# mikel-zhobro/pytorch3d_pointops

Measured on AMD Instinct MI355X. Metric: Mpoint-pairs/s (+ %HBM roofline) knn_points B=32 N=65536 K=16 @1/2/4/8 GPU, higher is better.
Workload: dtype f32; 1 GPU; knn_points B=32 N=M=65536 K=16 D=3 fp32 per GPU (BASELINE.json configs[1]); splitmix64 uniform [0,1)^3 clouds, p1 != p2, full lengths, norm=2; clouds_per_gpu=32, clouds_total=32

## Files before the change

### pytorch3d_pointops_amd/csrc/grid.h

```cpp
#pragma once
#include <float.h>
#include <math.h>

#include "knn_grid.h"

namespace pointops {

constexpr int kGMax = 1024;
constexpr int kEdgeStride = kGMax + 2;
constexpr int kGridWave = 64;
constexpr int kNumXcd = 8;
constexpr int kCoarseMax = 1024;
constexpr int kCrowdedMax = 64;
constexpr int kFineLogMax = 12;
constexpr int kOrderG = 16, kOrderBins = kOrderG * kOrderG * kOrderG;
constexpr int kSortedPad = 32;

inline int lane_search_workgroups(int64_t N, int P1) {
  const int64_t chunks = (N * ceil_div(P1, kGridWave) + 7) / 8 * 8;
  return (int)(chunks < 2048 ? 2048 : (chunks > (1 << 20) ? (1 << 20) : chunks));
}

struct GridCloud {
  float lo[3];
// ... 2 lines not shown
  int ncell;
  int len1, len2;
  int use_grid;
  int same;
  int mshift, nmicro;
};

struct RefinedCell {
  int start, count;
  int s;
  int pool_off;
  float lo[3], scale[3];
};

struct GridWs {
  GridCloud* cloud;
  int* chunk_prefix;
  float* edges;
  int* cell_start;
  int* coarse_count;
  int* bin_of;
  int* bin_first;
  int* nbins;
  int* coarse_cursor;
  int* coarse_start;
  float4* sorted;
  int* coarse_ticket;
  int* crowded_count;
  int* crowded_list;
  int* fine_count;
  int* prank;
  int* qrank;
  float4* qtmp;
  float4* qsorted;
  int* order_table;
  int* fb_count;
  int* fb_list;
  unsigned* fb_kth;
  int* fb2_count;
  int* fb2_list;
  int* fb3_count;
  int* fb3_list;
  unsigned* bbox;
  float* bbox_part;
  int* grid_flag;
  int* refine_ref;
  RefinedCell* rdesc;
  int* rcount;
  int* pool;
  int* pool_top;
  float4* sorted_tmp;
  int* box_count;
  int* box_list;
  int rdesc_cap, pool_cap;
  float c_target;
  int cell_cap;
  int ball;
};

struct GridBuild {
  float c_target;
  float h_min;
  float ball_radius;
  int ball_K;
  float ball_factor;
  bool same;
  int refine;
};

constexpr int kRefineMaxS = 32;

__host__ __device__ inline int refine_threshold(float c_target) {
  const float r = 28.0f * c_target;
  return r < 64.0f ? 64 : (int)r;
}
constexpr int kDeferFactor = 4;

__device__ __forceinline__ int sub_of(float x, float lo, float scale, int s) {
  const float t = (x - lo) * scale;
  int c = (t < (float)s) ? (int)t : s - 1;
  if (!(t >= 0.0f)) c = 0;
  return c;
}

size_t grid_carve(GridWs* ws, char* base, int64_t N, int64_t P1, int64_t P2, float c_target, bool ball = false);
int grid_build(const KnnArgs& a, const GridWs& ws, const GridBuild& b);
int grid_build_queries(const KnnArgs& a, const GridWs& ws, bool same, int level);
int grid_refine(const KnnArgs& a, const GridWs& ws);

__device__ __forceinline__ int cell_of(float x, float lo, float inv_h, int G) {
  const float t = (x - lo) * inv_h;
  int c = (t < (float)G) ? (int)t : G - 1;
  if (!(t >= 0.0f)) c = 0;
  return c;
}
__device__ __forceinline__ unsigned fkey(float f) {
  const unsigned u = __float_as_uint(f);
  return (u & 0x80000000u) ? ~u : (u | 0x80000000u);
}
__device__ __forceinline__ float funkey(unsigned k) {
  return __uint_as_float((k & 0x80000000u) ? (k & 0x7fffffffu) : ~k);
}
__device__ __forceinline__ float prev_float(float x) { return funkey(fkey(x) - 1u); }

template <int D>
__device__ __forceinline__ void load_point3(const float* __restrict__ p, float& x, float& y, float& z) {
  x = p[0];
  y = D > 1 ? p[1] : 0.0f;
  z = D > 2 ? p[2] : 0.0f;
}

__device__ __forceinline__ void point_cells(const GridCloud& g, float x, float y, float z, int& cx, int& cy,
                                            int& cz) {
  cx = cell_of(x, g.lo[0], g.inv_h, g.G[0]);
  cy = cell_of(y, g.lo[1], g.inv_h, g.G[1]);
  cz = cell_of(z, g.lo[2], g.inv_h, g.G[2]);
}
__device__ __forceinline__ int cell_index(const GridCloud& g, int cx, int cy, int cz) {
  return (cz * g.G[1] + cy) * g.G[0] + cx;
}
__device__ __forceinline__ int cell_id(const GridCloud& g, float x, float y, float z) {
  int cx, cy, cz;
  point_cells(g, x, y, z, cx, cy, cz);
  return cell_index(g, cx, cy, cz);
}

__device__ __forceinline__ int clamp_len(int64_t len, int P) {
  const int l = (int)len;
  return l < 0 ? 0 : (l > P ? P : l);
}

template <int BLOCK, typename Fn>
__device__ __forceinline__ void for_each4(const float4* __restrict__ src, int count, Fn fn) {
  for (int i0 = 0; i0 < count; i0 += 4 * BLOCK) {
    float4 p[4];
#pragma unroll
    for (int u = 0; u < 4; ++u) {
      const int j = i0 + u * BLOCK + (int)threadIdx.x;
      p[u] = j < count ? src[j] : make_float4(0.0f, 0.0f, 0.0f, 0.0f);
    }
#pragma unroll
    for (int u = 0; u < 4; ++u) {
      const int j = i0 + u * BLOCK + (int)threadIdx.x;
      fn(p[u], j, j < count);
    }
  }
}

template <int NORM>
__device__ __forceinline__ float face_bound(float t) {
  return NORM == 1 ? t : t * t;
}

template <int D, int NORM>
__device__ __forceinline__ float point_dist(float qx, float qy, float qz, const float4 c) {
  float d;
  if (NORM == 1) {
    d = __builtin_fabsf(qx - c.x);
    if (D > 1) d = d + __builtin_fabsf(qy - c.y);
    if (D > 2) d = d + __builtin_fabsf(qz - c.z);
  } else {
    const float dx = qx - c.x;
    d = dx * dx;
    if (D > 1) {
      const float dy = qy - c.y;
      d = d + dy * dy;
    }
    if (D > 2) {
      const float dz = qz - c.z;
      d = d + dz * dz;
    }
  }
  return d;
}

template <int NORM>
__device__ __forceinline__ float box_lower_bound(const GridCloud& g, const float* __restrict__ ed, float qx, float qy,
// ... 53 lines not shown
```

### pytorch3d_pointops_amd/csrc/grid_build.hip

```cpp
#include <stdlib.h>

#include "grid.h"
#include "wave.h"

namespace pointops {

constexpr int kSetupBlock = 1024;
constexpr int kCoarsePoints = 1024;

__device__ __forceinline__ int64_t coarse_row(int n, int set) { return ((int64_t)n * 2 + set) * (kCoarseMax + 1); }

__device__ __forceinline__ void reset_set_state(const GridWs& ws, int n, int set) {
  const int tid = threadIdx.x;
  if (tid == 0) {
    ws.coarse_ticket[n * 2 + set] = 0;
    ws.crowded_count[n * 2 + set] = 0;
    ws.nbins[n * 2 + set] = 0;
  }
  for (int t = tid; t < kCoarseMax + 1; t += kSetupBlock) {
    ws.coarse_count[coarse_row(n, set) + t] = 0;
    ws.coarse_cursor[coarse_row(n, set) + t] = 0;
  }
}
__device__ __forceinline__ void reset_query_state(const GridWs& ws, int n) {
// ... 175 lines not shown
    if (ok && any_active && !one_cell) {
      for (int d = 0; d < 3; ++d)
        if (active[d]) h = fmaxf(h, e[d] * (1.0f / ((float)kGMax - 0.5f)));
      for (int it = 0; it < 64; ++it) {
        inv_h = 1.0f / h;
        if (!(inv_h > 0.0f && inv_h <= FLT_MAX)) {
          ok = false;
          break;
        }
        long long cells = 1;
        for (int d = 0; d < 3; ++d) {
          G[d] = 1;
          if (active[d]) {
            const float t = e[d] * inv_h;
            G[d] = (t < (float)kGMax) ? (int)t + 1 : kGMax;
            if (G[d] < 1) G[d] = 1;
          }
          cells *= G[d];
        }
        if (cells <= (long long)ws.cell_cap && cells <= ((long long)kCoarseMax << kFineLogMax)) break;
        h *= 1.2599211f;
      }
      if ((long long)G[0] * G[1] * G[2] > (long long)ws.cell_cap ||
          (long long)G[0] * G[1] * G[2] > ((long long)kCoarseMax << kFineLogMax))
        ok = false;
    }
    for (int d = 0; d < 3; ++d) {
      g.lo[d] = lo[d];
      g.G[d] = G[d];
      s_hi[d] = hi[d];
    }
    g.inv_h = inv_h;
    g.ncell = G[0] * G[1] * G[2];
    g.len1 = len1;
    g.len2 = len2;
    g.mshift = 0;
    while (((g.ncell - 1) >> g.mshift) + 1 > kCoarseMax) ++g.mshift;
    g.nmicro = ((g.ncell - 1) >> g.mshift) + 1;
    if (g.mshift > kFineLogMax) ok = false;
    g.use_grid = ok ? 1 : 0;
    g.same = same;
    s_g = g;
    ws.cloud[n] = g;
    const float qnan = __uint_as_float(0x7fc00000u);
    ws.sorted[(int64_t)n * (P2 + kSortedPad) + P2] = make_float4(qnan, qnan, qnan, 0.0f);
    ws.grid_flag[n] = g.use_grid;
    ws.rcount[n] = 0;
    ws.pool_top[n] = 0;
  }
  reset_set_state(ws, n, 0);
  reset_query_state(ws, n);
  __syncthreads();
  if (s_g.use_grid) {
    float* __restrict__ ed = ws.edges + (int64_t)n * 3 * kEdgeStride;
    for (int t = tid; t < 3 * kEdgeStride; t += kSetupBlock) {
      const int d = t / kEdgeStride, c = t - d * kEdgeStride;
      const int G = s_g.G[d];
      ed[t] = (c <= G) ? edge_bisect(c, s_g.lo[d], s_hi[d], s_g.inv_h, G) : __builtin_inff();
    }
  }
}


__device__ void grid_chunk_prefix(const GridWs& ws, int N) {
  const int lane = threadIdx.x & (kWave - 1);
  int acc = 0;
  if (lane == 0) ws.chunk_prefix[0] = 0;
  for (int n0 = 0; n0 < N; n0 += kWave) {
    const int n = n0 + lane;
    int items = 0;
    if (n < N) {
      const GridCloud g = ws.cloud[n];
      if (g.use_grid) items = (g.len1 + kGridWave - 1) / kGridWave;
    }
    const int inc = wave_inclusive_sum(items);
    if (n < N) ws.chunk_prefix[n + 1] = acc + inc;
    acc += __shfl(inc, kWave - 1, kWave);
  }
}

constexpr int kPartBlock = 1024;
constexpr int kCountPerThread = 16;
constexpr int kScatterPerThread = 4;
constexpr int kSortBlock = 256;
constexpr int kHashBits = 12, kHashSlots = 1 << kHashBits, kHashProbes = 8;
constexpr int kCrowded = 8192;
constexpr int kCrowdedSlice = 4096;
constexpr int kFineMax = 1 << kFineLogMax;
static_assert(kCoarseMax == kPartBlock, "the count launch's last tile scans one micro-bin per thread");

__device__ __forceinline__ void unsearched_row(const GridWs& ws, const GridCloud& g, int n, int i, int P, int K,
                                               int64_t* __restrict__ idxs, float* __restrict__ dists) {
  if (i < P && i >= g.len1) {
    int64_t* __restrict__ zi = idxs + ((int64_t)n * P + i) * K;
    float* __restrict__ zd = dists + ((int64_t)n * P + i) * K;
    const int64_t pad = ws.ball ? -1 : 0;
    for (int k = 0; k < K; ++k) {
      zi[k] = pad;
      zd[k] = 0.0f;
    }
  } else if (i < g.len1 && !g.use_grid && !ws.ball) {
    const int pos = atomicAdd(ws.fb2_count + n, 1);
    ws.fb2_list[(int64_t)n * P + pos] = i;
  }
}

__device__ __forceinline__ void bin_cells(const GridCloud& g, const int* bfirst, int b, int& f0, int& nf) {
  f0 = bfirst[b] << g.mshift;
  nf = min((bfirst[b + 1] - bfirst[b]) << g.mshift, g.ncell - f0);
}

// ... 361 lines not shown
  }
}

static int grid_cell_cap(int64_t P2, float c_target) {
  const int64_t cells = (int64_t)ceil((double)P2 / (double)c_target);
  return (int)(2 * cells + 64);
}

size_t grid_carve(GridWs* ws, char* base, int64_t N, int64_t P1, int64_t P2, float c, bool ball) {
  const int cap = grid_cell_cap(P2, c);
  Carver cv(base);
  GridWs w;
  w.cell_cap = cap;
  w.cloud = (GridCloud*)cv.take(sizeof(GridCloud) * (size_t)N);
  w.chunk_prefix = (int*)cv.take(sizeof(int) * (size_t)(N + 1));
  w.edges = (float*)cv.take(sizeof(float) * (size_t)N * 3 * kEdgeStride);
  w.cell_start = (int*)cv.take(sizeof(int) * (size_t)N * (cap + 1));
  w.coarse_count = (int*)cv.take(sizeof(int) * (size_t)N * 2 * (kCoarseMax + 1));
  w.coarse_cursor = (int*)cv.take(sizeof(int) * (size_t)N * 2 * (kCoarseMax + 1));
  w.coarse_start = (int*)cv.take(sizeof(int) * (size_t)N * 2 * (kCoarseMax + 1));
  w.bin_of = (int*)cv.take(sizeof(int) * (size_t)N * 2 * (kCoarseMax + 1));
  w.bin_first = (int*)cv.take(sizeof(int) * (size_t)N * 2 * (kCoarseMax + 1));
  w.nbins = (int*)cv.take(sizeof(int) * (size_t)N * 2);
  w.coarse_ticket = (int*)cv.take(sizeof(int) * (size_t)N * 2);
  w.crowded_count = (int*)cv.take(sizeof(int) * (size_t)N * 2);
  w.crowded_list = (int*)cv.take(sizeof(int) * (size_t)N * 2 * kCrowdedMax);
  w.fine_count = (int*)cv.take(sizeof(int) * (size_t)N * 2 * cap);
  w.prank = (int*)cv.take(sizeof(int) * (size_t)N * (size_t)P2);
  w.qrank = (int*)cv.take(sizeof(int) * (size_t)N * (size_t)P1);
  w.order_table = (int*)cv.take(ball ? sizeof(int) * (size_t)N * (size_t)((P1 + 2047) / 2048) * kOrderBins : 0);
  w.sorted = (float4*)cv.take(sizeof(float4) * (size_t)N * (size_t)(P2 + kSortedPad));
  w.qsorted = (float4*)cv.take(sizeof(float4) * (size_t)N * (size_t)P1);
  w.fb_count = (int*)cv.take(sizeof(int) * (size_t)N);
  w.fb_list = (int*)cv.take(sizeof(int) * (size_t)N * (size_t)P1);
  w.fb_kth = (unsigned*)cv.take(sizeof(unsigned) * (size_t)N * (size_t)P1);
  w.fb2_count = (int*)cv.take(sizeof(int) * (size_t)N);
  w.fb2_list = (int*)cv.take(sizeof(int) * (size_t)N * (size_t)P1);
  w.fb3_count = (int*)cv.take(sizeof(int) * (size_t)N);
  w.fb3_list = (int*)cv.take(sizeof(int) * (size_t)N * (size_t)P1);
  w.bbox = (unsigned*)cv.take(sizeof(unsigned) * (size_t)N * 8);
  w.bbox_part = (float*)cv.take(sizeof(float) * (size_t)N * 6 * (size_t)((P2 + 2047) / 2048));
  w.grid_flag = (int*)cv.take(sizeof(int) * (size_t)N);
  w.qtmp = (float4*)cv.take(sizeof(float4) * (size_t)N * (size_t)P1);
  w.rdesc_cap = (int)(P2 / 64 + 1);
  w.pool_cap = (int)(4 * P2 + 64);
  w.refine_ref = (int*)cv.take(sizeof(int) * (size_t)N * cap);
  w.rdesc = (RefinedCell*)cv.take(sizeof(RefinedCell) * (size_t)N * (size_t)w.rdesc_cap);
  w.rcount = (int*)cv.take(sizeof(int) * (size_t)N);
  w.pool = (int*)cv.take(sizeof(int) * (size_t)N * (size_t)w.pool_cap);
  w.pool_top = (int*)cv.take(sizeof(int) * (size_t)N);
  w.sorted_tmp = (float4*)cv.take(sizeof(float4) * (size_t)N * (size_t)P2);
  w.box_count = (int*)cv.take(sizeof(int) * (size_t)N);
  w.box_list = (int*)cv.take(sizeof(int) * (size_t)N * (size_t)P1);
  w.c_target = c;
  w.ball = 0;
  if (ws) *ws = w;
  return cv.off;
}

template <int D>
static void build_d(const KnnArgs& a, const GridWs& ws, int sets_mode, int refine) {
  const bool same = sets_mode == 0;
  const unsigned sets = sets_mode == 2 ? 2u : 1u;
  const int zbase = sets_mode == 1 ? 1 : 0;
  const int64_t pmax = same ? a.P2 : sets_mode == 1 ? a.P1 : (a.P2 > a.P1 ? a.P2 : a.P1);
  auto part = [&](auto scatter, auto queries) {
    hipLaunchKernelGGL((grid_partition_kernel<D, scatter, queries>),
                       dim3((unsigned)ceil_div(pmax, kPartBlock * (scatter ? kScatterPerThread : kCountPerThread)),
                            (unsigned)a.N, sets),
                       dim3(kPartBlock), 0, a.stream, a.p2, a.P2, a.p1, a.P1, a.K, ws, zbase, a.idxs, a.dists);
  };
  if (same) {
    part(std::false_type{}, std::false_type{});
    part(std::true_type{}, std::false_type{});
  } else {
    part(std::false_type{}, std::true_type{});
    part(std::true_type{}, std::true_type{});
  }
  const int64_t bins = pmax / kCoarsePoints + ws.cell_cap / kFineMax + 2;
  int64_t wgs = 8192 / (a.N * (int64_t)sets);
  wgs = wgs < 16 ? 16 : (wgs > kCoarseMax ? kCoarseMax : wgs);
  wgs = wgs > bins ? bins : wgs;
  hipLaunchKernelGGL(grid_sort_kernel, dim3((unsigned)wgs, (unsigned)a.N, sets), dim3(kSortBlock), 0, a.stream, ws,
                     (int)a.P1, (int)a.P2, refine, zbase);
}

__global__ __launch_bounds__(kSetupBlock) void grid_requery_kernel(const int64_t* __restrict__ lengths1, int P1, int same,
                                                                GridWs ws) {
  const int n = blockIdx.x, tid = threadIdx.x;
  if (tid == 0) {
    ws.cloud[n].len1 = clamp_len(lengths1[n], P1);
    ws.cloud[n].same = same;
  }
  reset_query_state(ws, n);
}

__global__ __launch_bounds__(kPartBlock) void grid_pad_prefix_kernel(GridWs ws, int P1, int K, int64_t* __restrict__ idxs,
                                                                  float* __restrict__ dists) {
  const int n = blockIdx.y, tid = threadIdx.x;
  if (blockIdx.x == 0 && blockIdx.y == 0 && tid < kWave) grid_chunk_prefix(ws, (int)gridDim.y);
  const GridCloud g = ws.cloud[n];
  if (g.len1 >= P1 && g.use_grid) return;
  constexpr int kTile = kPartBlock * kCountPerThread;
  for (int r = 0; r < kCountPerThread; ++r)
    unsearched_row(ws, g, n, blockIdx.x * kTile + r * kPartBlock + tid, P1, K, idxs, dists);
}

int grid_build_queries(const KnnArgs& a, const GridWs& ws, bool same, int level) {
  hipLaunchKernelGGL(grid_requery_kernel, dim3((unsigned)a.N), dim3(kSetupBlock), 0, a.stream, a.l1, a.P1, same ? 1 : 0,
                     ws);
  if (same || level >= 2) {
    hipLaunchKernelGGL(grid_pad_prefix_kernel, dim3((unsigned)ceil_div(a.P1, kPartBlock * kCountPerThread), (unsigned)a.N),
                       dim3(kPartBlock), 0, a.stream, ws, a.P1, a.K, a.idxs, a.dists);
  } else {
    with_exact<3>(Ints<1, 2, 3>{}, a.D, [&](auto D) { build_d<D>(a, ws, 1, -1); });
  }
  return check_launch("grid build (queries)");
}

int grid_build(const KnnArgs& a, const GridWs& ws, const GridBuild& b) {
  const int bbox_slots = (int)ceil_div(a.P2, kBboxTile);
  hipLaunchKernelGGL(grid_bbox_kernel, dim3((unsigned)bbox_slots, (unsigned)a.N), dim3(kBboxBlock), 0, a.stream, a.p2,
                     a.l2, a.P2, a.D, ws.bbox_part);
  hipLaunchKernelGGL(grid_setup_kernel, dim3((unsigned)a.N), dim3(kSetupBlock), 0, a.stream, a.p2, a.l1, a.l2, a.P1,
                     a.P2, a.D, b.c_target, b.h_min, b.ball_radius, b.ball_K, b.ball_factor, b.same ? 1 : 0, bbox_slots,
                     ws);
  with_exact<3>(Ints<1, 2, 3>{}, a.D, [&](auto D) { build_d<D>(a, ws, b.same ? 0 : 2, b.refine); });
  return check_launch("grid build");
}

}
```

### pytorch3d_pointops_amd/csrc/grid_refine.hip

```cpp
#include "grid.h"
#include "wave.h"

namespace pointops {

constexpr int kRefineBlock = 1024;
constexpr int kRefineWgs = 8;

template <int D>
__global__ __launch_bounds__(kRefineBlock) void grid_refine_build_kernel(GridWs ws, int P2) {
  extern __shared__ int s_hist[];
  __shared__ double s_red[kRefineBlock / kWave][6];
  __shared__ float s_lo[3], s_scale[3];
  __shared__ int s_wsum[kRefineBlock / kWave];
  const int n = blockIdx.y;
  const int tid = threadIdx.x, lane = tid & (kWave - 1), wave = tid / kWave;
  int nref = ws.rcount[n];
  if (nref > ws.rdesc_cap) nref = ws.rdesc_cap;
  float4* __restrict__ rec = ws.sorted + (int64_t)n * (P2 + kSortedPad);
  float4* __restrict__ tmp = ws.sorted_tmp + (int64_t)n * P2;
  for (int r = blockIdx.x; r < nref; r += gridDim.x) {
    RefinedCell* __restrict__ dp = ws.rdesc + (int64_t)n * ws.rdesc_cap + r;
    const int start = dp->start, count = dp->count, s = dp->s;
    if (count <= 0) continue;
    const int nsub = s * s * s;
    double acc[6] = {0, 0, 0, 0, 0, 0};
    for_each4<kRefineBlock>(rec + start, count, [&](const float4 p, int, bool live) {
      if (!live) return;
      const double v[3] = {p.x, p.y, p.z};
#pragma unroll
      for (int d = 0; d < D; ++d) {
        acc[d] += v[d];
        acc[3 + d] += v[d] * v[d];
      }
    });
#pragma unroll
    for (int k = 0; k < 6; ++k) acc[k] = wave_sum(acc[k]);
    __syncthreads();
    if (lane == 0) {
#pragma unroll
      for (int k = 0; k < 6; ++k) s_red[wave][k] = acc[k];
    }
    __syncthreads();
    if (tid < 3) {
      float lo = 0.0f, scale = 0.0f;
      if (tid < D) {
        double sx = 0, sxx = 0;
        for (int w = 0; w < kRefineBlock / kWave; ++w) {
          sx += s_red[w][tid];
          sxx += s_red[w][3 + tid];
        }
        const double mean = sx / count;
        const double var = sxx / count - mean * mean;
        const double sig = var > 0 ? sqrt(var) : 0.0;
        const double half = 2.2 * sig;
        lo = (float)(mean - half);
        const float width = (float)(2.0 * half);
        scale = (width > 0.0f && width <= FLT_MAX) ? (float)s / width : 0.0f;
        if (!(scale > 0.0f && scale <= FLT_MAX)) scale = 0.0f;
        if (!(fabsf(lo) <= FLT_MAX)) {
          lo = 0.0f;
          scale = 0.0f;
        }
      }
      s_lo[tid] = lo;
      s_scale[tid] = scale;
      dp->lo[tid] = lo;
      dp->scale[tid] = scale;
    }
    for (int b = tid; b < nsub; b += kRefineBlock) s_hist[b] = 0;
    __syncthreads();
    const float lx = s_lo[0], ly = s_lo[1], lz = s_lo[2], kx = s_scale[0], ky = s_scale[1], kz = s_scale[2];
    auto sub_index = [&](const float4 p) {
      const int ix = sub_of(p.x, lx, kx, s);
      const int iy = D > 1 ? sub_of(p.y, ly, ky, s) : 0;
      const int iz = D > 2 ? sub_of(p.z, lz, kz, s) : 0;
      return (iz * s + iy) * s + ix;
    };
    for_each4<kRefineBlock>(rec + start, count, [&](const float4 p, int, bool live) {
      if (live) atomicAdd(&s_hist[sub_index(p)], 1);
    });
    __syncthreads();
    int* __restrict__ table = ws.pool + (int64_t)n * ws.pool_cap + dp->pool_off;
    const int per = (nsub + kRefineBlock - 1) / kRefineBlock;
    const int b0 = tid * per, b1 = min(b0 + per, nsub);
    int sum = 0;
    for (int b = b0; b < b1; ++b) sum += s_hist[b];
    int total;
    int run = block_exclusive_sum<kRefineBlock / kWave>(sum, s_wsum, total);
    for (int b = b0; b < b1; ++b) {
      const int cnt = s_hist[b];
      table[b] = run;
      s_hist[b] = run;
      run += cnt;
    }
    if (tid == kRefineBlock - 1) table[nsub] = count;
    __syncthreads();
    for_each4<kRefineBlock>(rec + start, count, [&](const float4 p, int, bool live) {
      if (live) tmp[start + atomicAdd(&s_hist[sub_index(p)], 1)] = p;
    });
    __threadfence_block();
    __syncthreads();
    for_each4<kRefineBlock>(tmp + start, count, [&](const float4 p, int i, bool live) {
      if (live) rec[start + i] = p;
    });
  }
}

int grid_refine(const KnnArgs& a, const GridWs& ws) {
  const size_t lds = sizeof(int) * (size_t)kRefineMaxS * kRefineMaxS * kRefineMaxS;
  const int64_t per_cloud = 256 / (a.N > 0 ? a.N : 1);
  const dim3 grid((unsigned)(per_cloud < kRefineWgs ? kRefineWgs : (per_cloud > 64 ? 64 : per_cloud)), (unsigned)a.N);
  const int rc = with_exact<3>(Ints<1, 2, 3>{}, a.D, [&](auto D) {
    static bool attr[64] = {false};
    int dev = -1;
    const bool known = hipGetDevice(&dev) == hipSuccess && dev >= 0 && dev < 64;
    if (!known || !attr[dev]) {
      if (hipFuncSetAttribute(reinterpret_cast<const void*>(grid_refine_build_kernel<D>),
                              hipFuncAttributeMaxDynamicSharedMemorySize, (int)lds) != hipSuccess)
        return check_launch("grid refine attribute");
      if (known) attr[dev] = true;
    }
    hipLaunchKernelGGL((grid_refine_build_kernel<D>), grid, dim3(kRefineBlock), lds, a.stream, ws, a.P2);
    return POINTOPS_OK;
  });
  if (rc != POINTOPS_OK) return rc;
  return check_launch("grid refine");
}

}
```

### pytorch3d_pointops_amd/csrc/knn_grid.hip

```cpp
#include "debug.h"
#include "grid.h"
#include "knn_grid_search.h"

namespace pointops {

static int grid_kc(int K) { return with_bucket(kGridKC, K, [](auto KC) { return KC.value; }); }

static float knn_cell_target(int K) {
  const int kc = grid_kc(K);
  float c = (kc >= 8 ? 0.4f : 0.625f) * (float)K;
  c *= (float)debug_knob_f("grid_c_scale", 1.0);
  return c < 1.0f ? 1.0f : c;
}

size_t knn_grid_workspace_bytes(int64_t N, int64_t P1, int64_t P2, int64_t K) {
  return grid_carve(nullptr, nullptr, N < 32768 ? N : 32768, P1, P2, knn_cell_target((int)K));
}

static bool grid_quad_mode(int64_t queries, int kc) {
  const long k = debug_knob("grid_quad", -1);
  return k >= 0 ? k != 0 : queries >= (kc >= 32 ? (1 << 18) : (1 << 20));
}

constexpr int64_t kGridBatchSlice = 32768;

int64_t knn_grid_max_points() { return kGridMaxPointsBig; }

static int knn_grid_run_slice(const KnnArgs& a, int norm, void* workspace, int reuse) {
  GridWs ws;
  const float c = knn_cell_target(a.K);
  grid_carve(&ws, (char*)workspace, a.N, a.P1, a.P2, c);
  GridBuild b{};
  b.c_target = c;
  b.same = a.p1 == a.p2 && a.l1 == a.l2 && a.P1 == a.P2 && debug_knob("grid_same", 1) != 0;
  b.refine = (debug_knob("grid_refine", 1) != 0 && a.K <= 64) ? 1 : 0;
  int rc;
  if (reuse > 0) {
    if ((rc = grid_build_queries(a, ws, b.same, reuse)) != POINTOPS_OK) return rc;
  } else {
    if ((rc = grid_build(a, ws, b)) != POINTOPS_OK) return rc;
    if (b.refine && (rc = grid_refine(a, ws)) != POINTOPS_OK) return rc;
  }
  if (a.K > 64) {
    grid_search_wsort(a, ws, norm);
    rc = check_launch("knn_points_idx(grid, long lists)");
    if (rc != POINTOPS_OK) return rc;
    KnnArgs fa = a;
    fa.qlist = ws.fb2_list;
    fa.qcount = ws.fb2_count;
    if ((rc = launch_knn_wide(fa, norm, 1, nullptr)) != POINTOPS_OK) return rc;
    return check_launch("knn_points_idx(grid fallback)");
  }
  const int kc = grid_kc(a.K);
  const bool quad = kc <= 32 && grid_quad_mode(a.N * (int64_t)a.P1, kc);
  const bool big = a.P2 > kGridMaxPoints || debug_knob("grid_big", 0) != 0;
  with_exact<3>(Ints<1, 2, 3>{}, a.D, [&](auto D) {
    (big ? grid_search<D, kRunBitsBig> : grid_search<D, kRunBitsStd>)(a, ws, norm, kc, quad);
  });
  rc = check_launch("knn_points_idx(grid)");
  if (rc != POINTOPS_OK) return rc;
  KnnArgs fa = a;
  fa.qlist = ws.fb2_list;
  fa.qcount = ws.fb2_count;
  if (a.K <= 32) launch_knn_bruteforce(fa, norm);
  else if ((rc = launch_knn_wide(fa, norm, 1, nullptr)) != POINTOPS_OK) return rc;
  return check_launch("knn_points_idx(grid fallback)");
}

int knn_grid_run(const KnnArgs& a, int norm, void* workspace, int reuse) {
  POINTOPS_REQUIRE(a.P2 <= kGridMaxPointsBig, "knn_points_idx(grid): P2 must be <= 2^24 - 16");
  if (a.N <= kGridBatchSlice) return knn_grid_run_slice(a, norm, workspace, reuse);
  for (int64_t n0 = 0; n0 < a.N; n0 += kGridBatchSlice) {
    KnnArgs s = a;
    const bool same_pts = a.p1 == a.p2, same_len = a.l1 == a.l2;
    s.N = a.N - n0 < kGridBatchSlice ? a.N - n0 : kGridBatchSlice;
    s.p1 = a.p1 + n0 * (int64_t)a.P1 * a.D;
    s.p2 = same_pts ? s.p1 : a.p2 + n0 * (int64_t)a.P2 * a.D;
    s.l1 = a.l1 + n0;
    s.l2 = same_len ? s.l1 : a.l2 + n0;
    s.idxs = a.idxs + n0 * (int64_t)a.P1 * a.K;
    s.dists = a.dists + n0 * (int64_t)a.P1 * a.K;
    const int rc = knn_grid_run_slice(s, norm, workspace, 0);
    if (rc != POINTOPS_OK) return rc;
  }
  return POINTOPS_OK;
}

}

extern "C" int pointops_knn_grid_fallback_counts(const void* workspace, int64_t N, int64_t P1, int64_t P2,
                                                 int64_t K, int32_t* counts, void* stream) {
  using namespace pointops;
  POINTOPS_REQUIRE(workspace != nullptr && counts != nullptr && N > 0 && N <= 32768, "knn_grid_fallback_counts: bad arguments");
  GridWs ws;
  grid_carve(&ws, (char*)workspace, N, P1, P2, knn_cell_target((int)K));
  if (hipMemcpyAsync(counts + N, ws.fb2_count, sizeof(int) * (size_t)N, hipMemcpyDeviceToDevice,
                     (hipStream_t)stream) != hipSuccess)
    return check_launch("knn_grid_fallback_counts");
  if (hipMemcpyAsync(counts, ws.fb_count, sizeof(int) * (size_t)N, hipMemcpyDeviceToDevice,
                     (hipStream_t)stream) != hipSuccess)
    return check_launch("knn_grid_fallback_counts");
  return POINTOPS_OK;
}

namespace pointops {
__global__ void grid_stats_kernel(GridWs ws, int N, int32_t* __restrict__ stats) {
  const int n = blockIdx.x * blockDim.x + threadIdx.x;
  if (n >= N) return;
// ... 30 lines not shown
```

### pytorch3d_pointops_amd/csrc/knn_grid_search.h

```cpp
#pragma once
#include "debug.h"
#include "grid.h"
#include "knn_common.h"
#include "sort_net.h"
#include "wave.h"

#include <type_traits>

namespace pointops {

template <int KC>
__device__ __forceinline__ void write_row_f64(const TopKF64<KC>& top, int K, int len2, int64_t* __restrict__ orow_i,
                                              float* __restrict__ orow_d, bool vec16) {
  write_row<KC>(top, K, len2, orow_i, orow_d, vec16);
}

constexpr int kLaneRows = 9;

template <int KC>
struct LaneCfg {
  static constexpr bool kUseQueue = KC >= 8;
  static constexpr int kQueueCap = 16;
  static constexpr int kQueueLds = KC <= 16 ? 15 : 16;
#ifndef POINTOPS_LANE_GROUP
// ... 70 lines not shown
    for (int u = u0; u < u0 + kSub; ++u) c[u] = record(off, u);
    __builtin_amdgcn_sched_barrier(0);
#pragma unroll
    for (int t = 0; t < kSub; ++t) {
      const bool valid = 16 * STRIDE * (u0 + t) < crem;
      if (kUseQueue) {
        if (valid && __float_as_uint(dd[t]) <= thr) {
          s_queue[qn] = TopKF64<KC>::make(dd[t], ii[t]);
          qn += kGridWave;
        }
      } else if (valid && __float_as_uint(dd[t]) <= min(top.worst_bits(), thr0)) {
        top.insert(TopKF64<KC>::make(dd[t], ii[t]));
      }
    }
  };
  if constexpr (kUseQueue) {
    static_assert(G == kSub && kQueueCap >= 2 * kSub, "queue geometry");
    bool more = __any(crem > 0);
    while (more) {
      bool full;
      do {
        advance();
        part(std::integral_constant<int, 0>{});
        crem = rem;
        more = __any(crem > 0);
        full = __any(qn > lane + (kQueueLds - kSub) * kGridWave);
      } while (!full && more);
      double qk[kQueueCap];
#pragma unroll
      for (int t = 0; t < kQueueCap; ++t) qk[t] = t < kQueueLds ? qbase[t * kGridWave] : TopKF64<KC>::empty();
#pragma unroll
      for (int t = 0; t < kQueueLds; ++t) qbase[t * kGridWave] = TopKF64<KC>::empty();
      bitonic_sort<kQueueCap>(qk);
      constexpr int kMeet = KC < kQueueCap ? KC : kQueueCap;
#pragma unroll
      for (int t = 0; t < kMeet; ++t) top.key[KC - 1 - t] = kmin(top.key[KC - 1 - t], qk[t]);
      bitonic_merge<KC>(top.key);
      qn = lane;
      thr = min(top.worst_bits(), thr0);
    }
  } else {
    static_assert(G == kSub, "direct-insert variants take one part per group");
    while (__any(crem > 0)) {
      advance();
      part(std::integral_constant<int, 0>{});
      crem = rem;
    }
  }
}

template <int D, int KC, int NORM, int RB>
__global__ __launch_bounds__(kGridWave, KC > 32 ? 2 : 1) void knn_grid_lane_kernel(
    const float* __restrict__ p1, const GridCloud* __restrict__ clouds, const int* __restrict__ chunk_prefix,
    const float* __restrict__ edges, const int* __restrict__ cell_start, const float4* __restrict__ sorted,
    const float4* __restrict__ qsorted, int* __restrict__ fb_count, int* __restrict__ fb_list,
    unsigned* __restrict__ fb_kth, int* __restrict__ box_count, int* __restrict__ box_list, int defer_limit,
    int uncertified_to_box, int cell_cap, int P1, int P2, int K, int N, int vec16, int64_t* __restrict__ idxs,
    float* __restrict__ dists) {
  using Cfg = LaneCfg<KC>;
  constexpr bool kUseQueue = Cfg::kUseQueue;
  constexpr int kQueueCap = Cfg::kQueueLds;
  constexpr int kSub = Cfg::kSub;
  constexpr int G = Cfg::kGroup;
  constexpr int kRunBits = RB, kRunMax = (1 << RB) - 1;
  static_assert(G % kSub == 0 && G <= kSortedPad, "group geometry");
  __shared__ double s_queue[kUseQueue ? kQueueCap * kGridWave : 1];
  __shared__ unsigned s_rows[kLaneRows + 1][kGridWave];

  const int lane = threadIdx.x;
  const int total = chunk_prefix[N];
  if (kUseQueue) {
#pragma unroll
    for (int t = 0; t < kQueueCap; ++t) s_queue[t * kGridWave + lane] = TopKF64<KC>::empty();
  }
  unsigned* const rows = &s_rows[0][0];
  const int xcd = blockIdx.x % kNumXcd, per_xcd = (total + kNumXcd - 1) / kNumXcd;
  for (int j = blockIdx.x / kNumXcd; j < per_xcd; j += gridDim.x / kNumXcd) {
    const int item = xcd * per_xcd + j;
    if (item >= total) break;
    const int n = item_cloud(chunk_prefix, N, item, (P1 + kGridWave - 1) / kGridWave);
    const GridCloud g = clouds[n];
    const int c0 = (item - chunk_prefix[n]) * kGridWave;
    const bool active = c0 + lane < g.len1;
    const float4* __restrict__ sp = sorted + (int64_t)n * (P2 + kSortedPad);
    int qi = 0;
    float qx = 0.0f, qy = 0.0f, qz = 0.0f;
    if (active) {
      const float4 q = (g.same ? sp : qsorted + (int64_t)n * P1)[c0 + lane];
      qx = q.x;
      qy = q.y;
      qz = q.z;
      qi = __float_as_int(q.w);
    }
    int cx, cy, cz;
    point_cells(g, qx, qy, qz, cx, cy, cz);
    const int X0 = max(cx - 1, 0), X1 = min(cx + 1, g.G[0] - 1);
    const int Y0 = max(cy - 1, 0), Y1 = min(cy + 1, g.G[1] - 1);
    const int Z0 = max(cz - 1, 0), Z1 = min(cz + 1, g.G[2] - 1);
    const int* __restrict__ cstart = cell_start + (int64_t)n * (cell_cap + 1);

    const float* __restrict__ ed = edges + (int64_t)n * 3 * kEdgeStride;
    const float edge[6] = {ed[X0], ed[X1 + 1], ed[kEdgeStride + Y0], ed[kEdgeStride + Y1 + 1], ed[2 * kEdgeStride + Z0],
                           ed[2 * kEdgeStride + Z1 + 1]};
    constexpr int kDz[kLaneRows] = {0, 0, 0, -1, 1, -1, -1, 1, 1};
    constexpr int kDy[kLaneRows] = {0, -1, 1, 0, 0, -1, 1, -1, 1};
    int row_s[kLaneRows], row_e[kLaneRows];
#pragma unroll
    for (int r = 0; r < kLaneRows; ++r) {
      const int z = min(max(cz + kDz[r], 0), g.G[2] - 1), y = min(max(cy + kDy[r], 0), g.G[1] - 1);
      const int rowbase = (z * g.G[1] + y) * g.G[0];
      row_s[r] = cstart[rowbase + X0];
      row_e[r] = cstart[rowbase + X1 + 1];
    }

    bool whole;
    const float lb = box_lower_bound_from<NORM>(g, edge, qx, qy, qz, X0, X1, Y0, Y1, Z0, Z1, whole);
    const unsigned thr0 = seed_threshold(lb, whole);

    bool overlong = false;
    {
      int cnt = 0;
      int total = 0;
#pragma unroll
      for (int r = 0; r < kLaneRows; ++r) {
        const int z = cz + kDz[r], y = cy + kDy[r];
        const int s = row_s[r], e = row_e[r];
        const bool listed = active & (z >= 0) & (z < g.G[2]) & (y >= 0) & (y < g.G[1]) & (e > s);
        if (listed) {
          overlong = overlong || e - s > kRunMax;
          total += e - s;
          rows[lane + cnt] = ((unsigned)s << kRunBits) | (unsigned)min(e - s, kRunMax);
          cnt += kGridWave;
        }
      }
      overlong = overlong || total > defer_limit;
      if (overlong) cnt = 0;
#pragma unroll
      for (int r = 0; r <= kLaneRows; ++r) {
        if (r * kGridWave >= cnt) s_rows[r][lane] = 0u;
      }
    }
    TopKF64<KC> top;
    top.init();
    lane_walk<D, KC, NORM, kLaneRows, RB>((const char*)sp, rows, lane, s_queue, qx, qy, qz, thr0, top);

    const unsigned kth_bits = top.kth_bits(K);
    const bool full = kth_bits < 0x7f800000u;
    const bool ok = !overlong && (whole || (full && __uint_as_float(kth_bits) < lb));
    if (active) {
      if (ok) {
        const int64_t row = (int64_t)n * P1 + qi;
        write_row_f64<KC>(top, K, g.len2, idxs + row * K, dists + row * K, vec16 != 0);
      } else if (overlong || uncertified_to_box) {
        const int pos = atomicAdd(box_count + n, 1);
        box_list[(int64_t)n * P1 + pos] = qi;
      } else {
        const int pos = atomicAdd(fb_count + n, 1);
        fb_list[(int64_t)n * P1 + pos] = qi;
        int m = 0;
#pragma unroll
        for (int t = 0; t < KC; ++t) m += (unsigned)__double2hiint(top.key[t]) < 0x7f800000u ? 1 : 0;
        const float est = m > 0 ? lb * __powf(fmaxf((float)K / (float)m, 1.0f), NORM == 1 ? 0.33333f : 0.66667f) * 1.3f
                                : __builtin_inff();
        fb_kth[(int64_t)n * P1 + pos] = __float_as_uint(est);
      }
    }
  }
}

#ifndef POINTOPS_QUAD_LANES
#define POINTOPS_QUAD_LANES 4
#endif
constexpr int kQuadLanes = POINTOPS_QUAD_LANES;
static_assert(kQuadLanes == 4 || kQuadLanes == 8, "lanes per query");
constexpr int kQuadRows = 25;
constexpr int kQuadQueries = kGridWave / kQuadLanes;
constexpr int kQuadMaxRecords = 1024;
__device__ constexpr signed char kQuadDy[32] = {0, 0, 0, -1, 1, -1, -1, 1, 1, 0, 0, -2, 2, -1, 1, -1, 1, -2, -2, 2, 2, -2, -2, 2, 2, 0, 0, 0, 0, 0, 0, 0};
__device__ constexpr signed char kQuadDz[32] = {0, -1, 1, 0, 0, -1, 1, -1, 1, -2, 2, 0, 0, -2, -2, 2, 2, -1, 1, -1, 1, -2, 2, -2, 2, 0, 0, 0, 0, 0, 0, 0};

constexpr int kDppXor1 = 0xB1, kDppXor2 = 0x4E, kDppHalfMirror = 0x141;

template <int CTRL>
__device__ __forceinline__ double dpp_f64(double v) {
  const int lo = __builtin_amdgcn_mov_dpp(__double2loint(v), CTRL, 0xf, 0xf, true);
  const int hi = __builtin_amdgcn_mov_dpp(__double2hiint(v), CTRL, 0xf, 0xf, true);
  return __hiloint2double(hi, lo);
}

template <int KC, int CTRL>
__device__ __forceinline__ void dpp_merge(TopKF64<KC>& top) {
  double o[KC];
#pragma unroll
  for (int t = 0; t < KC; ++t) o[t] = dpp_f64<CTRL>(top.key[t]);
  if constexpr (KC >= 2) {
#pragma unroll
    for (int t = 0; t < KC; ++t) top.key[t] = kmin(top.key[t], o[KC - 1 - t]);
    bitonic_merge<KC>(top.key);
  } else {
    top.key[0] = kmin(top.key[0], o[0]);
  }
}

template <int D, int KC, int NORM, int RB>
__global__ __launch_bounds__(kGridWave, KC >= 32 ? 2 : 1) void knn_grid_quad_kernel(
// ... 208 lines not shown
        }
      }
      if (giveup) {
        if (lane == 0) {
          const int pos = atomicAdd(fb2_count + n, 1);
          fb2_list[(int64_t)n * P1 + pos] = qi;
        }
        break;
      }
      double mine = TopKF64<KC>::empty(), kth = TopKF64<KC>::empty();
      for (int k = 0; k < kvalid; ++k) {
        double m = top.key[0];
#pragma unroll
        for (int off = kWave / 2; off > 0; off >>= 1) {
          const int hi = __shfl_xor(__double2hiint(m), off, kWave);
          const int lo = __shfl_xor(__double2loint(m), off, kWave);
          m = kmin(m, __hiloint2double(hi, lo));
        }
        if (lane == k) mine = m;
        kth = m;
        if (__double_as_longlong(top.key[0]) == __double_as_longlong(m)) {
#pragma unroll
          for (int s2 = 0; s2 + 1 < KC; ++s2) top.key[s2] = top.key[s2 + 1];
          top.key[KC - 1] = TopKF64<KC>::empty();
        }
      }
      const unsigned kth_bits = (unsigned)__double2hiint(kth);
      const bool full = kvalid == K && kth_bits < 0x7f800000u;
      if (whole || (full && __uint_as_float(kth_bits) < lb)) {
        if (lane < K) {
          const bool ok = lane < kvalid;
          idxs[row * K + lane] = ok ? (int64_t)__double2loint(mine) : 0;
          dists[row * K + lane] = ok ? __int_as_float(__double2hiint(mine)) : 0.0f;
        }
        done = true;
      }
    }
  }
}

template <int D, int KC, int NORM, int RB>
static void launch_grid_box(const KnnArgs& a, const GridWs& ws, bool quad);

static inline bool long_lists_to_box(const KnnArgs& a) {
  const long k = debug_knob("grid_long_box", -1);
  return k >= 0 ? k != 0 : a.N * (int64_t)a.P1 >= (3LL << 19);
}

template <int D, int KC, int NORM, int RB>
static void launch_grid_passes(const KnnArgs& a, const GridWs& ws, bool quad) {
  const int wgs = lane_search_workgroups(a.N, a.P1);
  hipLaunchKernelGGL((knn_grid_lane_kernel<D, KC, NORM, RB>), dim3((unsigned)wgs), dim3(kGridWave), 0, a.stream, a.p1,
                     (const GridCloud*)ws.cloud, (const int*)ws.chunk_prefix, (const float*)ws.edges,
                     (const int*)ws.cell_start, (const float4*)ws.sorted, (const float4*)ws.qsorted, ws.fb_count,
                     ws.fb_list, ws.fb_kth, ws.box_count, ws.box_list, kDeferFactor * refine_threshold(ws.c_target),
                     (KC > 32 && long_lists_to_box(a)) ? 1 : 0, ws.cell_cap, a.P1, a.P2, a.K, (int)a.N,
                     row_stores_16b(a) ? 1 : 0, a.idxs, a.dists);
  if constexpr (KC <= 32) if (quad) {
    int64_t wx = a.P1 / (32 * kQuadQueries);
    wx = wx < 8 ? 8 : wx > 4096 ? 4096 : wx;
    hipLaunchKernelGGL((knn_grid_quad_kernel<D, KC, NORM, RB>), dim3((unsigned)wx, (unsigned)a.N), dim3(kGridWave), 0,
                       a.stream, a.p1, (const GridCloud*)ws.cloud, (const float*)ws.edges, (const int*)ws.cell_start,
                       (const float4*)ws.sorted, (const int*)ws.fb_count, (const int*)ws.fb_list,
                       (const unsigned*)ws.fb_kth, ws.fb3_count, ws.fb3_list, ws.box_count, ws.box_list, ws.cell_cap, a.P1,
                       a.P2, a.K, row_stores_16b(a) ? 1 : 0, a.idxs, a.dists);
  }
  launch_grid_box<D, KC, NORM, RB>(a, ws, quad);
  hipLaunchKernelGGL((knn_grid_wave_kernel<D, KC, NORM>), dim3(kWaveKernelWgsPerCloud, (unsigned)a.N),
                     dim3(kWaveKernelBlock), 0, a.stream, a.p1, (const GridCloud*)ws.cloud, (const float*)ws.edges,
                     (const int*)ws.cell_start, (const float4*)ws.sorted,
                     (const int*)(quad ? ws.fb3_count : ws.fb_count), (const int*)(quad ? ws.fb3_list : ws.fb_list),
                     ws.fb2_count, ws.fb2_list, ws.cell_cap, a.P1, a.P2, a.K, quad ? 4 : 2, a.idxs, a.dists);
}

constexpr Ints<1, 2, 4, 8, 16, 32, 64> kGridKC{};

template <int D, int RB>
void grid_search(const KnnArgs& a, const GridWs& ws, int norm, int kc, bool quad) {
  with_exact<2>(Ints<1, 2>{}, norm, [&](auto NORM) {
    with_bucket(kGridKC, kc, [&](auto KC) {
      launch_grid_passes<D, KC, NORM, RB>(a, ws, KC <= 32 && quad);
    });
  });
}

extern template void grid_search<1, kRunBitsStd>(const KnnArgs&, const GridWs&, int, int, bool);
extern template void grid_search<2, kRunBitsStd>(const KnnArgs&, const GridWs&, int, int, bool);
extern template void grid_search<3, kRunBitsStd>(const KnnArgs&, const GridWs&, int, int, bool);
extern template void grid_search<1, kRunBitsBig>(const KnnArgs&, const GridWs&, int, int, bool);
extern template void grid_search<2, kRunBitsBig>(const KnnArgs&, const GridWs&, int, int, bool);
extern template void grid_search<3, kRunBitsBig>(const KnnArgs&, const GridWs&, int, int, bool);

}
```

Baseline: 262.5 million Mpoint-pairs/s.

## Precompute per-cell row-run words and edge pairs for the lane search

Adds a per-cell table of packed (start,len) row runs covering the x-neighbourhood and a per-cell float2 edge-pair table, built during setup/refine (or in a small extra kernel). The lane search kernel then loads nine packed words and three float2 edges instead of eighteen cell_start loads and six scattered edge loads, and computes the overlong/total checks branch-free. This trades extra workspace memory and build work for fewer dependent gather loads in the hot search kernel. Also pins K/vec16 to scalar registers via asm.

```diff
diff --git a/pytorch3d_pointops_amd/csrc/grid.h b/pytorch3d_pointops_amd/csrc/grid.h
--- a/pytorch3d_pointops_amd/csrc/grid.h
+++ b/pytorch3d_pointops_amd/csrc/grid.h
@@ -78,6 +78,8 @@
   float4* sorted_tmp;
   int* box_count;
   int* box_list;
+  unsigned* row_run;
+  float2* edge_pair;
   int rdesc_cap, pool_cap;
   float c_target;
   int cell_cap;
@@ -112,7 +114,8 @@
 size_t grid_carve(GridWs* ws, char* base, int64_t N, int64_t P1, int64_t P2, float c_target, bool ball = false);
 int grid_build(const KnnArgs& a, const GridWs& ws, const GridBuild& b);
 int grid_build_queries(const KnnArgs& a, const GridWs& ws, bool same, int level);
-int grid_refine(const KnnArgs& a, const GridWs& ws);
+int grid_refine(const KnnArgs& a, const GridWs& ws, int run_bits);
+int grid_row_runs(const KnnArgs& a, const GridWs& ws, int run_bits);
 
 __device__ __forceinline__ int cell_of(float x, float lo, float inv_h, int G) {
   const float t = (x - lo) * inv_h;
@@ -149,6 +152,19 @@
   int cx, cy, cz;
   point_cells(g, x, y, z, cx, cy, cz);
   return cell_index(g, cx, cy, cz);
+}
+
+__device__ __forceinline__ void write_row_runs(const GridWs& ws, int n, int run_bits, int first, int step) {
+  const GridCloud g = ws.cloud[n];
+  if (!g.use_grid) return;
+  const int* __restrict__ cstart = ws.cell_start + (int64_t)n * (ws.cell_cap + 1);
+  unsigned* __restrict__ rr = ws.row_run + (int64_t)n * ws.cell_cap;
+  const int G0 = g.G[0], run_max = (1 << run_bits) - 1;
+  for (int c = first; c < g.ncell; c += step) {
+    const int x = c % G0;
+    const int s = cstart[c - (x > 0 ? 1 : 0)], e = cstart[c + (x < G0 - 1 ? 1 : 0) + 1];
+    rr[c] = ((unsigned)s << run_bits) | (unsigned)min(e - s, run_max);
+  }
 }
 
 __device__ __forceinline__ int clamp_len(int64_t len, int P) {
diff --git a/pytorch3d_pointops_amd/csrc/grid_build.hip b/pytorch3d_pointops_amd/csrc/grid_build.hip
--- a/pytorch3d_pointops_amd/csrc/grid_build.hip
+++ b/pytorch3d_pointops_amd/csrc/grid_build.hip
@@ -251,11 +251,20 @@
   reset_query_state(ws, n);
   __syncthreads();
   if (s_g.use_grid) {
+    __shared__ float s_ed[3 * kEdgeStride];
     float* __restrict__ ed = ws.edges + (int64_t)n * 3 * kEdgeStride;
     for (int t = tid; t < 3 * kEdgeStride; t += kSetupBlock) {
       const int d = t / kEdgeStride, c = t - d * kEdgeStride;
       const int G = s_g.G[d];
-      ed[t] = (c <= G) ? edge_bisect(c, s_g.lo[d], s_hi[d], s_g.inv_h, G) : __builtin_inff();
+      ed[t] = s_ed[t] = (c <= G) ? edge_bisect(c, s_g.lo[d], s_hi[d], s_g.inv_h, G) : __builtin_inff();
+    }
+    __syncthreads();
+    float2* __restrict__ ep = ws.edge_pair + (int64_t)n * 3 * kEdgeStride;
+    for (int t = tid; t < 3 * kEdgeStride; t += kSetupBlock) {
+      const int d = t / kEdgeStride, c = t - d * kEdgeStride;
+      const int G = s_g.G[d];
+      if (c < G)
+        ep[3 * c + d] = make_float2(s_ed[d * kEdgeStride + max(c - 1, 0)], s_ed[d * kEdgeStride + min(c + 1, G - 1) + 1]);
     }
   }
 }
@@ -723,6 +732,8 @@
   w.sorted_tmp = (float4*)cv.take(sizeof(float4) * (size_t)N * (size_t)P2);
   w.box_count = (int*)cv.take(sizeof(int) * (size_t)N);
   w.box_list = (int*)cv.take(sizeof(int) * (size_t)N * (size_t)P1);
+  w.row_run = (unsigned*)cv.take(sizeof(unsigned) * (size_t)N * cap);
+  w.edge_pair = (float2*)cv.take(sizeof(float2) * (size_t)N * 3 * kEdgeStride);
   w.c_target = c;
   w.ball = 0;
   if (ws) *ws = w;
@@ -789,6 +800,18 @@
   return check_launch("grid build (queries)");
 }
 
+constexpr int kRowRunBlock = 256;
+__global__ __launch_bounds__(kRowRunBlock) void grid_row_runs_kernel(GridWs ws, int run_bits) {
+  write_row_runs(ws, blockIdx.y, run_bits, blockIdx.x * kRowRunBlock + threadIdx.x, gridDim.x * kRowRunBlock);
+}
+
+int grid_row_runs(const KnnArgs& a, const GridWs& ws, int run_bits) {
+  const int64_t wx = ceil_div((int64_t)ws.cell_cap, 4 * kRowRunBlock);
+  hipLaunchKernelGGL(grid_row_runs_kernel, dim3((unsigned)(wx > 1024 ? 1024 : wx), (unsigned)a.N), dim3(kRowRunBlock), 0,
+                     a.stream, ws, run_bits);
+  return check_launch("grid row runs");
+}
+
 int grid_build(const KnnArgs& a, const GridWs& ws, const GridBuild& b) {
   const int bbox_slots = (int)ceil_div(a.P2, kBboxTile);
   hipLaunchKernelGGL(grid_bbox_kernel, dim3((unsigned)bbox_slots, (unsigned)a.N), dim3(kBboxBlock), 0, a.stream, a.p2,
diff --git a/pytorch3d_pointops_amd/csrc/grid_refine.hip b/pytorch3d_pointops_amd/csrc/grid_refine.hip
--- a/pytorch3d_pointops_amd/csrc/grid_refine.hip
+++ b/pytorch3d_pointops_amd/csrc/grid_refine.hip
@@ -7,13 +7,14 @@
 constexpr int kRefineWgs = 8;
 
 template <int D>
-__global__ __launch_bounds__(kRefineBlock) void grid_refine_build_kernel(GridWs ws, int P2) {
+__global__ __launch_bounds__(kRefineBlock) void grid_refine_build_kernel(GridWs ws, int P2, int run_bits) {
   extern __shared__ int s_hist[];
   __shared__ double s_red[kRefineBlock / kWave][6];
   __shared__ float s_lo[3], s_scale[3];
   __shared__ int s_wsum[kRefineBlock / kWave];
   const int n = blockIdx.y;
   const int tid = threadIdx.x, lane = tid & (kWave - 1), wave = tid / kWave;
+  if (run_bits > 0) write_row_runs(ws, n, run_bits, blockIdx.x * kRefineBlock + tid, gridDim.x * kRefineBlock);
   int nref = ws.rcount[n];
   if (nref > ws.rdesc_cap) nref = ws.rdesc_cap;
   float4* __restrict__ rec = ws.sorted + (int64_t)n * (P2 + kSortedPad);
@@ -106,7 +107,7 @@
   }
 }
 
-int grid_refine(const KnnArgs& a, const GridWs& ws) {
+int grid_refine(const KnnArgs& a, const GridWs& ws, int run_bits) {
   const size_t lds = sizeof(int) * (size_t)kRefineMaxS * kRefineMaxS * kRefineMaxS;
   const int64_t per_cloud = 256 / (a.N > 0 ? a.N : 1);
   const dim3 grid((unsigned)(per_cloud < kRefineWgs ? kRefineWgs : (per_cloud > 64 ? 64 : per_cloud)), (unsigned)a.N);
@@ -120,7 +121,7 @@
         return check_launch("grid refine attribute");
       if (known) attr[dev] = true;
     }
-    hipLaunchKernelGGL((grid_refine_build_kernel<D>), grid, dim3(kRefineBlock), lds, a.stream, ws, a.P2);
+    hipLaunchKernelGGL((grid_refine_build_kernel<D>), grid, dim3(kRefineBlock), lds, a.stream, ws, a.P2, run_bits);
     return POINTOPS_OK;
   });
   if (rc != POINTOPS_OK) return rc;
diff --git a/pytorch3d_pointops_amd/csrc/knn_grid.hip b/pytorch3d_pointops_amd/csrc/knn_grid.hip
--- a/pytorch3d_pointops_amd/csrc/knn_grid.hip
+++ b/pytorch3d_pointops_amd/csrc/knn_grid.hip
@@ -34,12 +34,16 @@
   b.c_target = c;
   b.same = a.p1 == a.p2 && a.l1 == a.l2 && a.P1 == a.P2 && debug_knob("grid_same", 1) != 0;
   b.refine = (debug_knob("grid_refine", 1) != 0 && a.K <= 64) ? 1 : 0;
+  const bool big = a.P2 > kGridMaxPoints || debug_knob("grid_big", 0) != 0;
+  const int run_bits = big ? kRunBitsBig : kRunBitsStd;
   int rc;
   if (reuse > 0) {
     if ((rc = grid_build_queries(a, ws, b.same, reuse)) != POINTOPS_OK) return rc;
   } else {
     if ((rc = grid_build(a, ws, b)) != POINTOPS_OK) return rc;
-    if (b.refine && (rc = grid_refine(a, ws)) != POINTOPS_OK) return rc;
+    if (b.refine) rc = grid_refine(a, ws, run_bits);
+    else if (a.K <= 64) rc = grid_row_runs(a, ws, run_bits);
+    if (rc != POINTOPS_OK) return rc;
   }
   if (a.K > 64) {
     grid_search_wsort(a, ws, norm);
@@ -53,7 +57,6 @@
   }
   const int kc = grid_kc(a.K);
   const bool quad = kc <= 32 && grid_quad_mode(a.N * (int64_t)a.P1, kc);
-  const bool big = a.P2 > kGridMaxPoints || debug_knob("grid_big", 0) != 0;
   with_exact<3>(Ints<1, 2, 3>{}, a.D, [&](auto D) {
     (big ? grid_search<D, kRunBitsBig> : grid_search<D, kRunBitsStd>)(a, ws, norm, kc, quad);
   });
diff --git a/pytorch3d_pointops_amd/csrc/knn_grid_search.h b/pytorch3d_pointops_amd/csrc/knn_grid_search.h
--- a/pytorch3d_pointops_amd/csrc/knn_grid_search.h
+++ b/pytorch3d_pointops_amd/csrc/knn_grid_search.h
@@ -146,17 +146,18 @@
 template <int D, int KC, int NORM, int RB>
 __global__ __launch_bounds__(kGridWave, KC > 32 ? 2 : 1) void knn_grid_lane_kernel(
     const float* __restrict__ p1, const GridCloud* __restrict__ clouds, const int* __restrict__ chunk_prefix,
-    const float* __restrict__ edges, const int* __restrict__ cell_start, const float4* __restrict__ sorted,
-    const float4* __restrict__ qsorted, int* __restrict__ fb_count, int* __restrict__ fb_list,
-    unsigned* __restrict__ fb_kth, int* __restrict__ box_count, int* __restrict__ box_list, int defer_limit,
-    int uncertified_to_box, int cell_cap, int P1, int P2, int K, int N, int vec16, int64_t* __restrict__ idxs,
-    float* __restrict__ dists) {
+    const float* __restrict__ edges, const int* __restrict__ cell_start, const unsigned* __restrict__ row_run,
+    const float2* __restrict__ edge_pair, const float4* __restrict__ sorted, const float4* __restrict__ qsorted,
+    int* __restrict__ fb_count, int* __restrict__ fb_list, unsigned* __restrict__ fb_kth, int* __restrict__ box_count,
+    int* __restrict__ box_list, int defer_limit, int uncertified_to_box, int cell_cap, int P1, int P2, int K, int N,
+    int vec16, int64_t* __restrict__ idxs, float* __restrict__ dists) {
   using Cfg = LaneCfg<KC>;
   constexpr bool kUseQueue = Cfg::kUseQueue;
   constexpr int kQueueCap = Cfg::kQueueLds;
   constexpr int kSub = Cfg::kSub;
   constexpr int G = Cfg::kGroup;
-  constexpr int kRunBits = RB, kRunMax = (1 << RB) - 1;
+  [[maybe_unused]] constexpr int kRunBits = RB;
+  constexpr int kRunMax = (1 << RB) - 1;
   static_assert(G % kSub == 0 && G <= kSortedPad, "group geometry");
   __shared__ double s_queue[kUseQueue ? kQueueCap * kGridWave : 1];
   __shared__ unsigned s_rows[kLaneRows + 1][kGridWave];
@@ -191,60 +192,94 @@
     const int X0 = max(cx - 1, 0), X1 = min(cx + 1, g.G[0] - 1);
     const int Y0 = max(cy - 1, 0), Y1 = min(cy + 1, g.G[1] - 1);
     const int Z0 = max(cz - 1, 0), Z1 = min(cz + 1, g.G[2] - 1);
-    const int* __restrict__ cstart = cell_start + (int64_t)n * (cell_cap + 1);
-
+
+#ifndef POINTOPS_LANE_ROW_TABLE
+#define POINTOPS_LANE_ROW_TABLE 1
+#endif
+#ifndef POINTOPS_LANE_EDGE_PAIRS
+#define POINTOPS_LANE_EDGE_PAIRS 1
+#endif
+#if POINTOPS_LANE_EDGE_PAIRS
+    const char* __restrict__ epb = (const char*)(edge_pair + (int64_t)n * 3 * kEdgeStride);
+    float2 ex = *(const float2*)(epb + __umul24((unsigned)cx, 24u));
+    float2 ey = *(const float2*)(epb + __umul24((unsigned)cy, 24u) + 8u);
+    float2 ez = *(const float2*)(epb + __umul24((unsigned)cz, 24u) + 16u);
+    float edge[6] = {ex.x, ex.y, ey.x, ey.y, ez.x, ez.y};
+#else
     const float* __restrict__ ed = edges + (int64_t)n * 3 * kEdgeStride;
     const float edge[6] = {ed[X0], ed[X1 + 1], ed[kEdgeStride + Y0], ed[kEdgeStride + Y1 + 1], ed[2 * kEdgeStride + Z0],
                            ed[2 * kEdgeStride + Z1 + 1]};
+#endif
     constexpr int kDz[kLaneRows] = {0, 0, 0, -1, 1, -1, -1, 1, 1};
     constexpr int kDy[kLaneRows] = {0, -1, 1, 0, 0, -1, 1, -1, 1};
-    int row_s[kLaneRows], row_e[kLaneRows];
-#pragma unroll
-    for (int r = 0; r < kLaneRows; ++r) {
-      const int z = min(max(cz + kDz[r], 0), g.G[2] - 1), y = min(max(cy + kDy[r], 0), g.G[1] - 1);
-      const int rowbase = (z * g.G[1] + y) * g.G[0];
-      row_s[r] = cstart[rowbase + X0];
-      row_e[r] = cstart[rowbase + X1 + 1];
-    }
+    const bool hy[3] = {cy > 0, true, cy < g.G[1] - 1}, hz[3] = {cz > 0, true, cz < g.G[2] - 1};
+    unsigned word[kLaneRows];
+#if POINTOPS_LANE_ROW_TABLE
+    {
+      const char* __restrict__ rrb = (const char*)(row_run + (int64_t)n * cell_cap);
+      const unsigned sy = 4u * (unsigned)g.G[0], sz = sy * (unsigned)g.G[1];
+      const unsigned own = __umul24(__umul24((unsigned)cz, (unsigned)g.G[1]) + (unsigned)cy, sy) + 4u * (unsigned)cx;
+      const unsigned oy[3] = {hy[0] ? 0u - sy : 0u, 0u, hy[2] ? sy : 0u};
+      const unsigned oz[3] = {hz[0] ? 0u - sz : 0u, 0u, hz[2] ? sz : 0u};
+#pragma unroll
+      for (int r = 0; r < kLaneRows; ++r) word[r] = *(const unsigned*)(rrb + (own + oz[kDz[r] + 1] + oy[kDy[r] + 1]));
+    }
+#else
+    {
+      const int* __restrict__ cstart = cell_start + (int64_t)n * (cell_cap + 1);
+#pragma unroll
+      for (int r = 0; r < kLaneRows; ++r) {
+        const int z = min(max(cz + kDz[r], 0), g.G[2] - 1), y = min(max(cy + kDy[r], 0), g.G[1] - 1);
+        const int rowbase = (z * g.G[1] + y) * g.G[0];
+        const int s = cstart[rowbase + X0], e = cstart[rowbase + X1 + 1];
+        word[r] = ((unsigned)s << kRunBits) | (unsigned)min(e - s, kRunMax);
+      }
+    }
+#endif
+
+#if POINTOPS_LANE_EDGE_PAIRS
+#pragma unroll
+    for (int t = 0; t < 6; ++t) asm volatile("" : "+v"(edge[t]));
+#endif
 
     bool whole;
     const float lb = box_lower_bound_from<NORM>(g, edge, qx, qy, qz, X0, X1, Y0, Y1, Z0, Z1, whole);
     const unsigned thr0 = seed_threshold(lb, whole);
 
-    bool overlong = false;
+    unsigned total = 0u, longest = 0u;
+#pragma unroll
+    for (int r = 0; r < kLaneRows; ++r) {
+      word[r] = (hz[kDz[r] + 1] && hy[kDy[r] + 1]) ? word[r] : 0u;
+      const unsigned len = word[r] & (unsigned)kRunMax;
+      total += len;
+      longest = max(longest, len);
+    }
+    const bool overlong = active && (longest == (unsigned)kRunMax || total > (unsigned)defer_limit);
+    const bool walks = active && !overlong;
     {
+#pragma unroll
+      for (int r = 0; r <= kLaneRows; ++r) s_rows[r][lane] = 0u;
       int cnt = 0;
-      int total = 0;
 #pragma unroll
       for (int r = 0; r < kLaneRows; ++r) {
-        const int z = cz + kDz[r], y = cy + kDy[r];
-        const int s = row_s[r], e = row_e[r];
-        const bool listed = active & (z >= 0) & (z < g.G[2]) & (y >= 0) & (y < g.G[1]) & (e > s);
-        if (listed) {
-          overlong = overlong || e - s > kRunMax;
-          total += e - s;
-          rows[lane + cnt] = ((unsigned)s << kRunBits) | (unsigned)min(e - s, kRunMax);
-          cnt += kGridWave;
-        }
-      }
-      overlong = overlong || total > defer_limit;
-      if (overlong) cnt = 0;
-#pragma unroll
-      for (int r = 0; r <= kLaneRows; ++r) {
-        if (r * kGridWave >= cnt) s_rows[r][lane] = 0u;
+        const bool listed = walks && (word[r] & (unsigned)kRunMax) != 0u;
+        rows[lane + cnt] = listed ? word[r] : 0u;
+        cnt += listed ? kGridWave : 0;
       }
     }
     TopKF64<KC> top;
     top.init();
     lane_walk<D, KC, NORM, kLaneRows, RB>((const char*)sp, rows, lane, s_queue, qx, qy, qz, thr0, top);
 
-    const unsigned kth_bits = top.kth_bits(K);
+    int Kc = K, vec16c = vec16;
+    asm volatile("" : "+s"(Kc), "+s"(vec16c));
+    const unsigned kth_bits = top.kth_bits(Kc);
     const bool full = kth_bits < 0x7f800000u;
     const bool ok = !overlong && (whole || (full && __uint_as_float(kth_bits) < lb));
     if (active) {
       if (ok) {
         const int64_t row = (int64_t)n * P1 + qi;
-        write_row_f64<KC>(top, K, g.len2, idxs + row * K, dists + row * K, vec16 != 0);
+        write_row_f64<KC>(top, Kc, g.len2, idxs + row * Kc, dists + row * Kc, vec16c != 0);
       } else if (overlong || uncertified_to_box) {
         const int pos = atomicAdd(box_count + n, 1);
         box_list[(int64_t)n * P1 + pos] = qi;
@@ -559,8 +594,9 @@
   const int wgs = lane_search_workgroups(a.N, a.P1);
   hipLaunchKernelGGL((knn_grid_lane_kernel<D, KC, NORM, RB>), dim3((unsigned)wgs), dim3(kGridWave), 0, a.stream, a.p1,
                      (const GridCloud*)ws.cloud, (const int*)ws.chunk_prefix, (const float*)ws.edges,
-                     (const int*)ws.cell_start, (const float4*)ws.sorted, (const float4*)ws.qsorted, ws.fb_count,
-                     ws.fb_list, ws.fb_kth, ws.box_count, ws.box_list, kDeferFactor * refine_threshold(ws.c_target),
+                     (const int*)ws.cell_start, (const unsigned*)ws.row_run, (const float2*)ws.edge_pair,
+                     (const float4*)ws.sorted, (const float4*)ws.qsorted, ws.fb_count, ws.fb_list, ws.fb_kth,
+                     ws.box_count, ws.box_list, kDeferFactor * refine_threshold(ws.c_target),
                      (KC > 32 && long_lists_to_box(a)) ? 1 : 0, ws.cell_cap, a.P1, a.P2, a.K, (int)a.N,
                      row_stores_16b(a) ? 1 : 0, a.idxs, a.dists);
   if constexpr (KC <= 32) if (quad) {
```

Result: no change. 264.2 million Mpoint-pairs/s (median of 6 runs) (+0.6%).
